# drscotthawley/signaltrain

Hardware: AMD Instinct MI355X
Metric: audio-frames/sec (train step) comp_4c 8192-sample windows @ 1/2/4/8 GPUs (higher is better)
Workload: dtype f32; 1 GPU; comp_4c synthetic, 8192-sample windows, batch 256/GPU, fp32 (BASELINE configs[1]); window=8192, frames_per_window=25, global_batch=256, parallelism=dp1

## Files before the change

### signaltrain_amd/csrc/st_ae.h

```cpp
#pragma once
#include "st_common.h"

namespace sta {

constexpr int NL = 9;
#ifndef ST_AE_ABLATE
#define ST_AE_ABLATE 0
#endif

struct AEOffsets { int w[NL]; int b[NL]; };

struct GroupWalk { int first, end, stride; };
__device__ __forceinline__ GroupWalk fwd_group_walk(const int ngroups, const int NW, const int wave)
{
    const int G = (int)gridDim.x, b = (int)blockIdx.x;
    if ((G & 7) == 0) {
        const int S = G >> 3, x = b & 7, slot = b >> 3;
        const int per = (ngroups + 7) >> 3;
        const int lo = x * per, hi = lo + per < ngroups ? lo + per : ngroups;
        return GroupWalk{lo + wave * S + slot, hi, S * NW};
    }
    return GroupWalk{wave * G + b, ngroups, G * NW};
}

struct CL {
    static constexpr int O0 = 64, O1 = 32, O2 = 16, O3 = 16, O4 = 16, O5 = 16, O6 = 32, O7 = 64, O8 = 16;
    static constexpr int I0 = 32, I1 = 64, I2 = 32, I3 = 16, I4 = 32, I5 = 16, I6 = 16, I7 = 32, I8 = 64;
    static constexpr int A0 = 0, A1 = A0 + O0 * I0, A2 = A1 + O1 * I1, A3 = A2 + O2 * I2, A4 = A3 + O3 * I3, A5 = A4 + O4 * I4,
                         A6 = A5 + O5 * I5, A7 = A6 + O6 * I6, A8 = A7 + O7 * I7, AEND = A8 + O8 * I8;
    static constexpr int B0 = AEND, B1 = B0 + O0, B2 = B1 + O1, B3 = B2 + O2, B4 = B3 + O3, B5 = B4 + O4, B6 = B5 + O5,
                         B7 = B6 + O6, B8 = B7 + O7, FWD_TOTAL = B8 + O8;
    static constexpr int G0 = FWD_TOTAL, G1 = G0 + O0 * I0, G2 = G1 + O1 * I1, G3 = G2 + O2 * I2, G4 = G3 + O3 * I3, G5 = G4 + O4 * I4,
                         G6 = G5 + O5 * I5, G7 = G6 + O6 * I6, G8 = G7 + O7 * I7, BWD_TOTAL = G8 + O8 * I8;
    static_assert(FWD_TOTAL % 4 == 0 && BWD_TOTAL % 4 == 0, "16-byte aligned regions");
};

constexpr int ae_max_elems(int l) { return l == 0 ? 64 * 32 : l == 1 ? 32 * 64 : l == 2 ? 16 * 32 : l == 3 ? 16 * 16 : l == 4 ? 16 * 32 :
                                           l == 5 ? 16 * 16 : l == 6 ? 32 * 16 : l == 7 ? 64 * 32 : 16 * 64; }
template <int NT>
struct AEParamRegs { float v[NL][(64 * 32 + NT - 1) / NT]; float bv[NL]; };

template <int NT>
__host__ __device__ __forceinline__ void ae_params_issue(AEParamRegs<NT>& r, const float* __restrict__ ae, const AEOffsets& go,
                                                const int T, const int OT, const int K, const int tid, const int l0, const int l1)
{
    const int out[NL] = {64, 32, 16, 16, 16, 16, 32, 64, OT};
    const int in[NL] = {T, 64, 32, 16, 16 + K, 16, 16, 32, 64};
#pragma unroll
    for (int l = 0; l < NL; ++l) {
        const bool on = l >= l0 && l < l1;
        const int n = on ? out[l] * in[l] : 0;
        const float* src = ae + go.w[l];
#pragma unroll
        for (int u = 0; u < (ae_max_elems(l) + NT - 1) / NT; ++u) { const int e = tid + u * NT; r.v[l][u] = src[e < n ? e : 0]; }
        r.bv[l] = ae[go.b[l] + (tid < out[l] ? tid : 0)];
    }
}
template <int BF> __device__ __forceinline__ unsigned short st_half_bits(const float v)
{
    if constexpr (BF == 2) { union { _Float16 h; unsigned short u; } p; p.h = (_Float16)v; return p.u; }
    else { union { __bf16 h; unsigned short u; } p; p.h = (__bf16)v; return p.u; }
}
template <int BF> __device__ __forceinline__ float st_half_to_float(const unsigned short b)
{
    if constexpr (BF == 2) { union { unsigned short u; _Float16 h; } p; p.u = b; return (float)p.h; }
    else return __uint_as_float((unsigned)b << 16);
}
template <int NT, int BF = 0>
__host__ __device__ __forceinline__ void ae_params_scatter(float* lds, const AEParamRegs<NT>& r, const int T, const int OT, const int K,
                                                  const int tid, const int l0, const int l1, const bool dgrad_images)
{
    const int out[NL] = {64, 32, 16, 16, 16, 16, 32, 64, OT};
    const int in[NL] = {T, 64, 32, 16, 16 + K, 16, 16, 32, 64};
    const int outp[NL] = {CL::O0, CL::O1, CL::O2, CL::O3, CL::O4, CL::O5, CL::O6, CL::O7, CL::O8};
    const int inp[NL] = {CL::I0, CL::I1, CL::I2, CL::I3, CL::I4, CL::I5, CL::I6, CL::I7, CL::I8};
    const int ao[NL] = {CL::A0, CL::A1, CL::A2, CL::A3, CL::A4, CL::A5, CL::A6, CL::A7, CL::A8};
    const int bo[NL] = {CL::B0, CL::B1, CL::B2, CL::B3, CL::B4, CL::B5, CL::B6, CL::B7, CL::B8};
    const int gi[NL] = {CL::G0, CL::G1, CL::G2, CL::G3, CL::G4, CL::G5, CL::G6, CL::G7, CL::G8};
#pragma unroll
    for (int l = 0; l < NL; ++l) {
        const bool on = l >= l0 && l < l1;
        const int IN = in[l], n = on ? out[l] * IN : 0, OP = outp[l], IP = inp[l];
#pragma unroll
        for (int u = 0; u < (ae_max_elems(l) + NT - 1) / NT; ++u) {
            const int e = tid + u * NT;
            if (e < n) {
                const int o = e / IN, i = e - o * IN;
                if constexpr (BF) {
                    const unsigned short hb = st_half_bits<BF>(r.v[l][u]);
                    reinterpret_cast<unsigned short*>(lds + ao[l])[(((i >> 2) * OP + o) << 2) + (i & 3)] = hb;
                    if (dgrad_images) reinterpret_cast<unsigned short*>(lds + gi[l])[(((o >> 2) * IP + i) << 2) + (o & 3)] = hb;
                } else {
                lds[ao[l] + (((i >> 2) * OP + o) << 2) + (i & 3)] = r.v[l][u];
                if (dgrad_images) lds[gi[l] + (((o >> 2) * IP + i) << 2) + (o & 3)] = r.v[l][u];
                }
            }
        }
        if (on && tid < out[l]) lds[bo[l] + tid] = r.bv[l];
    }
}
template <int NT, int BF = 0>
__device__ inline void ae_load_lds(float* lds, const float* __restrict__ ae, const AEOffsets& go, const int T, const int OT, const int K,
                                   const int tid, const int l0, const int l1, const bool dgrad_images)
{
    const int total = dgrad_images ? CL::BWD_TOTAL : CL::FWD_TOTAL;
#if ST_AE_ABLATE & 128
    for (int e = tid; e < total; e += NT) lds[e] = 0.f;
#else
    AEParamRegs<NT> r;
    ae_params_issue<NT>(r, ae, go, T, OT, K, tid, l0, l1);
    for (int e = tid; e < total; e += NT) lds[e] = 0.f;
    __syncthreads();
    ae_params_scatter<NT, BF>(lds, r, T, OT, K, tid, l0, l1, dgrad_images);
#endif
}
template <int NT, int BF = 0>
__device__ inline void ae_load_lds2(float* lds, const float* __restrict__ ae_m, const float* __restrict__ ae_p, const AEOffsets& go,
                                    const int T, const int OT, const int K, const int tid, const int l0, const int l1)
{
#if ST_AE_ABLATE & 128
    for (int e = tid; e < 2 * CL::FWD_TOTAL; e += NT) lds[e] = 0.f;
#else
    AEParamRegs<NT> rm, rp;
    ae_params_issue<NT>(rm, ae_m, go, T, OT, K, tid, l0, l1);
    ae_params_issue<NT>(rp, ae_p, go, T, OT, K, tid, l0, l1);
    for (int e = tid; e < 2 * CL::FWD_TOTAL; e += NT) lds[e] = 0.f;
    __syncthreads();
    ae_params_scatter<NT, BF>(lds, rm, T, OT, K, tid, l0, l1, false);
    ae_params_scatter<NT, BF>(lds + CL::FWD_TOTAL, rp, T, OT, K, tid, l0, l1, false);
#endif
}

constexpr int AE_IMG_DG = CL::BWD_TOTAL - CL::FWD_TOTAL;
__host__ __device__ constexpr int ae_img_fwd_floats(const int FP) { return 2 * CL::FWD_TOTAL + FP; }
__host__ __device__ constexpr int ae_img_floats(const int FP) { return ae_img_fwd_floats(FP) + 2 * AE_IMG_DG; }
struct AEImgJob { const float* ae[2]; float* img; AEOffsets go; int T, OT, K, F, FP; float expfac; int n, n_blk; };
__host__ __device__ __forceinline__ float ae_freq_weight(const float expfac, const int f) { return expf(expfac * (float)f); }
__host__ __device__ __forceinline__ void ae_img_build(const AEImgJob& j, const int p)
{
    if (p >= j.n) return;
    const int out[NL] = {64, 32, 16, 16, 16, 16, 32, 64, j.OT};
    const int in[NL] = {j.T, 64, 32, 16, 16 + j.K, 16, 16, 32, 64};
    const int outp[NL] = {CL::O0, CL::O1, CL::O2, CL::O3, CL::O4, CL::O5, CL::O6, CL::O7, CL::O8};
    const int inp[NL] = {CL::I0, CL::I1, CL::I2, CL::I3, CL::I4, CL::I5, CL::I6, CL::I7, CL::I8};
    const int ao[NL + 1] = {CL::A0, CL::A1, CL::A2, CL::A3, CL::A4, CL::A5, CL::A6, CL::A7, CL::A8, CL::AEND};
    const int bo[NL + 1] = {CL::B0, CL::B1, CL::B2, CL::B3, CL::B4, CL::B5, CL::B6, CL::B7, CL::B8, CL::FWD_TOTAL};
    float v = 0.f;
    const int q0 = p - 2 * CL::FWD_TOTAL;
    if (q0 >= 0 && q0 < j.FP) v = q0 < j.F ? ae_freq_weight(j.expfac, q0) : 0.f;
    else {
        const bool dg = q0 >= 0;
        const int net = dg ? (q0 - j.FP >= AE_IMG_DG) : (p >= CL::FWD_TOTAL);
        const int q = dg ? q0 - j.FP - net * AE_IMG_DG : p - net * CL::FWD_TOTAL;
        const float* __restrict__ ae = j.ae[net];
        if (!dg && q >= CL::AEND) {
#pragma unroll
            for (int l = 0; l < NL; ++l)
                if (q >= bo[l] && q < bo[l + 1]) { const int o = q - bo[l]; if (o < out[l]) v = ae[j.go.b[l] + o]; }
        } else {
#pragma unroll
            for (int l = 0; l < NL; ++l)
                if (q >= ao[l] && q < ao[l + 1]) {
                    const int s = (q - ao[l]) >> 2, lo = (q - ao[l]) & 3;
                    const int o = dg ? ((s / inp[l]) << 2) + lo : s % outp[l];
                    const int i = dg ? s % inp[l] : ((s / outp[l]) << 2) + lo;
                    if (o < out[l] && i < in[l]) v = ae[j.go.w[l] + o * in[l] + i];
                }
        }
    }
    j.img[p] = v;
}

#define ST_MFMA16(a, b, c) __builtin_amdgcn_mfma_f32_16x16x4f32((a), (b), (c), 0, 0, 0)

__device__ __forceinline__ float ldg32(const float* __restrict__ base, const unsigned elem)
{
    return *reinterpret_cast<const float*>(reinterpret_cast<const char*>(base) + (size_t)(elem << 2));
}
__device__ __forceinline__ void stg32(float* __restrict__ base, const unsigned elem, const float v)
{
    *reinterpret_cast<float*>(reinterpret_cast<char*>(base) + (size_t)(elem << 2)) = v;
}
#define ST_MUL24(a, b) __umul24((unsigned)(a), (unsigned)(b))

typedef short s16x4 __attribute__((ext_vector_type(4)));
typedef __bf16 bf16x4_t __attribute__((ext_vector_type(4)));
typedef _Float16 f16x4_t __attribute__((ext_vector_type(4)));
template <int BF>
__device__ __forceinline__ f32x4 mfma16h(const s16x4 a, const s16x4 b, const f32x4 c)
{
    if constexpr (BF == 2) {
        union { s16x4 s; f16x4_t h; } pa, pb; pa.s = a; pb.s = b;
        return __builtin_amdgcn_mfma_f32_16x16x16f16(pa.h, pb.h, c, 0, 0, 0);
    } else return __builtin_amdgcn_mfma_f32_16x16x16bf16_1k(a, b, c, 0, 0, 0);
}
#define ST_MFMA16B(a, b, c) mfma16h<BF>((a), (b), (c))
template <int BF>
__device__ __forceinline__ s16x4 pack_h4(f32x4 v)
{
    if constexpr (BF == 2) {
        union { f16x4_t h; s16x4 s; } p; p.h = __builtin_convertvector(v, f16x4_t); return p.s;
    } else {
        typedef __bf16 bf16x2_t __attribute__((ext_vector_type(2)));
        typedef float f32x2_t __attribute__((ext_vector_type(2)));
        union { bf16x2_t h; unsigned u; } lo, hi;
        lo.h = __builtin_convertvector((f32x2_t){v[0], v[1]}, bf16x2_t);
        hi.h = __builtin_convertvector((f32x2_t){v[2], v[3]}, bf16x2_t);
        union { unsigned u[2]; s16x4 s; } r; r.u[0] = lo.u; r.u[1] = hi.u; return r.s;
    }
}
#define pack_bf16x4(v) pack_h4<BF>(v)
template <int BF>
__device__ __forceinline__ float round_h(const float v)
{
    if constexpr (BF == 2) return (float)(_Float16)v;
    else {
        union { __bf16 h; unsigned short u; } p; p.h = (__bf16)v;
        union { unsigned u; float f; } q; q.u = (unsigned)p.u << 16; return q.f;
    }
}
#define bf16_rne(v) round_h<BF>(v)

template <int BF>
__device__ __forceinline__ f32x4 frag_read(const float* img, const int idx)
{
    if constexpr (BF) {
        typedef float f32x2_t __attribute__((ext_vector_type(2)));
        const f32x2_t lo = *reinterpret_cast<const f32x2_t*>(reinterpret_cast<const unsigned short*>(img) + idx);
        return __builtin_shufflevector(lo, lo, 0, 1, -1, -1);
    } else return *reinterpret_cast<const f32x4*>(img + idx);
}
__device__ __forceinline__ s16x4 frag_bits(const f32x4 v)
{
    typedef float f32x2_t __attribute__((ext_vector_type(2)));
    union { f32x2_t f; s16x4 s; } p; p.f = __builtin_shufflevector(v, v, 0, 1); return p.s;
}
template <int OUTP, int BF = 0>
__device__ __forceinline__ f32x4 frag_fwd(const float* img, const int ot, const int it, const int g, const int c)
{
    return frag_read<BF>(img, ((4 * it + g) * OUTP + 16 * ot + c) << 2);
}
template <int INP, int BF = 0>
__device__ __forceinline__ f32x4 frag_dgrad(const float* img, const int ot, const int it, const int g, const int c)
{
    return frag_read<BF>(img, ((4 * ot + g) * INP + 16 * it + c) << 2);
}

template <int NC, int OTL, int ITL, int OUTP, int BF = 0>
__device__ __forceinline__ void layer_fwd(const float* const (&W)[NC], const float* const (&bias)[NC],
                                          const f32x4 (&hin)[NC][ITL], f32x4 (&hout)[NC][OTL], const int g, const int c)
{
    s16x4 ph[NC][ITL];
    if constexpr (BF) {
#pragma unroll
        for (int ch = 0; ch < NC; ++ch)
#pragma unroll
            for (int it = 0; it < ITL; ++it) ph[ch][it] = pack_bf16x4(hin[ch][it]);
    }
#pragma unroll
    for (int ot = 0; ot < OTL; ++ot) {
        f32x4 acc[NC];
#pragma unroll
        for (int ch = 0; ch < NC; ++ch) acc[ch] = *reinterpret_cast<const f32x4*>(bias[ch] + 16 * ot + 4 * g);
#pragma unroll
        for (int it = 0; it < ITL; ++it) {
            f32x4 w[NC];
#pragma unroll
            for (int ch = 0; ch < NC; ++ch) w[ch] = frag_fwd<OUTP, BF>(W[ch], ot, it, g, c);
            if constexpr (BF) {
#pragma unroll
                for (int ch = 0; ch < NC; ++ch) acc[ch] = ST_MFMA16B(frag_bits(w[ch]), ph[ch][it], acc[ch]);
            } else {
#pragma unroll
                for (int r = 0; r < 4; ++r)
#pragma unroll
                    for (int ch = 0; ch < NC; ++ch) acc[ch] = ST_MFMA16(w[ch][r], hin[ch][it][r], acc[ch]);
            }
        }
#pragma unroll
        for (int ch = 0; ch < NC; ++ch) hout[ch][ot] = elu4(acc[ch]);
    }
}

template <int NC, int BF = 0>
__device__ __forceinline__ void layer5_fwd(const float* const (&lw)[NC], const f32x4 (&h4)[NC][1], const float (&kn)[4], const int KQ,
                                           f32x4 (&h5)[NC][1], const int g, const int c)
{
    f32x4 acc[NC], w[NC];
#pragma unroll
    for (int ch = 0; ch < NC; ++ch) { acc[ch] = *reinterpret_cast<const f32x4*>(lw[ch] + CL::B4 + 4 * g); w[ch] = frag_fwd<CL::O4, BF>(lw[ch] + CL::A4, 0, 0, g, c); }
    if constexpr (BF) {
#pragma unroll
        for (int ch = 0; ch < NC; ++ch) acc[ch] = ST_MFMA16B(frag_bits(w[ch]), pack_bf16x4(h4[ch][0]), acc[ch]);
    } else {
#pragma unroll
        for (int r = 0; r < 4; ++r)
#pragma unroll
            for (int ch = 0; ch < NC; ++ch) acc[ch] = ST_MFMA16(w[ch][r], h4[ch][0][r], acc[ch]);
    }
#pragma unroll
    for (int q = 0; q < 4; ++q)
        if (q < KQ) {
#pragma unroll
            for (int ch = 0; ch < NC; ++ch) {
                float wk;
                if constexpr (BF) wk = st_half_to_float<BF>(reinterpret_cast<const unsigned short*>(lw[ch] + CL::A4)[(((4 + q) * CL::O4 + c) << 2) + g]);
                else wk = lw[ch][CL::A4 + (((4 + q) * CL::O4 + c) << 2) + g];
                acc[ch] = ST_MFMA16(wk, BF ? bf16_rne(kn[q]) : kn[q], acc[ch]);
            }
        }
#pragma unroll
    for (int ch = 0; ch < NC; ++ch) h5[ch][0] = elu4(acc[ch]);
}

#define ST_W2(off_) {lw[0] + (off_), lw[1] + (off_)}

struct FwdIn { f32x4 v[2][2]; float tl[2][4]; float kn[4]; };

__device__ __forceinline__ void fwd_load_v(FwdIn& in, const float* __restrict__ mag, const float* __restrict__ phs,
                                           const int b, const int f, const bool fv, const int T, const int F, const int g)
{
    const unsigned base = ST_MUL24(ST_MUL24(b, T), F) + (unsigned)(fv ? f : 0);
#pragma unroll
// ... 275 lines not shown
#pragma unroll
        for (int it = 0; it < ITL; ++it) ph[it] = pack_bf16x4(hin[it]);
    }
#pragma unroll
    for (int ot = 0; ot < OTL; ++ot) {
        f32x4 acc = *reinterpret_cast<const f32x4*>(bias + 16 * ot + 4 * g);
#pragma unroll
        for (int it = 0; it < ITL; ++it) {
#if ST_AE_ABLATE & 32
            acc[0] += fr[ot * ITL + it][0] * hin[it][0];
#else
            if constexpr (BF) acc = ST_MFMA16B(frag_bits(fr[ot * ITL + it]), ph[it], acc);
            else {
#pragma unroll
                for (int r = 0; r < 4; ++r) acc = ST_MFMA16(fr[ot * ITL + it][r], hin[it][r], acc);
            }
#endif
        }
#if ST_AE_ABLATE & 8
#pragma unroll
        for (int r = 0; r < 4; ++r) hout[ot][r] = fmaxf(acc[r], 0.1f * acc[r]);
#else
        hout[ot] = elu4(acc);
#endif
    }
}
template <int TL>
__device__ __forceinline__ void to_T(float* scr, const f32x4 (&d)[TL], f32x4 (&t)[TL], const int g, const int c)
{
#if ST_AE_ABLATE & 16
#pragma unroll
    for (int k = 0; k < TL; ++k) t[k] = d[k];
    return;
#endif
#pragma unroll
    for (int k = 0; k < TL; ++k) *reinterpret_cast<f32x4*>(scr + k * 320 + c * 20 + 4 * g) = d[k];
#pragma unroll
    for (int k = 0; k < TL; ++k)
#pragma unroll
        for (int r = 0; r < 4; ++r) t[k][r] = scr[k * 320 + (4 * g + r) * 20 + c];
}

template <int BF> struct TTy { typedef f32x4 type; };
template <> struct TTy<1> { typedef s16x4 type; };
template <> struct TTy<2> { typedef s16x4 type; };
template <int TL, int BF>
__device__ __forceinline__ void to_Th(float* scr, const f32x4 (&d)[TL], typename TTy<BF>::type (&t)[TL], const int g, const int c)
{
    if constexpr (BF == 0) to_T<TL>(scr, d, t, g, c);
    else {
        short* hs = reinterpret_cast<short*>(scr);
#pragma unroll
        for (int k = 0; k < TL; ++k) *reinterpret_cast<s16x4*>(hs + k * 256 + c * 16 + 4 * g) = pack_h4<BF>(d[k]);
#pragma unroll
        for (int k = 0; k < TL; ++k)
            t[k] = __builtin_amdgcn_ds_read_tr16_b64_v4i16((s16x4 __attribute__((address_space(3)))*)(hs + k * 256 + (4 * g + (c >> 2)) * 16 + 4 * (c & 3)));
    }
}
template <int BF>
__device__ __forceinline__ typename TTy<BF>::type tt_splat(const float v)
{
    if constexpr (BF == 0) return (f32x4){v, v, v, v};
    else return pack_h4<BF>((f32x4){v, v, v, v});
}
template <int OTL, int ITL, int BF>
__device__ __forceinline__ void wgrad_regh(f32x4 (&dW)[OTL][ITL], float (&db)[OTL], const f32x4 (&daT)[OTL], const typename TTy<BF>::type (&hT)[ITL]);

template <int OTL, int ITL, int BF = 0>
__device__ __forceinline__ void dgradD_fr(const f32x4 (&fr)[ITL * OTL], const f32x4 (&da)[OTL], f32x4 (&dh)[ITL])
{
    s16x4 pd[OTL];
    if constexpr (BF) {
#pragma unroll
        for (int ot = 0; ot < OTL; ++ot) pd[ot] = pack_bf16x4(da[ot]);
    }
#pragma unroll
    for (int it = 0; it < ITL; ++it) {
        f32x4 acc = (f32x4){0.f, 0.f, 0.f, 0.f};
#pragma unroll
        for (int ot = 0; ot < OTL; ++ot) {
            if constexpr (BF) acc = ST_MFMA16B(frag_bits(fr[it * OTL + ot]), pd[ot], acc);
            else {
#pragma unroll
                for (int r = 0; r < 4; ++r) acc = ST_MFMA16(fr[it * OTL + ot][r], da[ot][r], acc);
            }
        }
        dh[it] = acc;
    }
}

template <int TL>
__device__ __forceinline__ void mul_elu_grad(f32x4 (&d)[TL], const f32x4 (&h)[TL])
{
#pragma unroll
    for (int t = 0; t < TL; ++t)
#pragma unroll
        for (int r = 0; r < 4; ++r) d[t][r] = __builtin_fmaf(d[t][r], __builtin_amdgcn_fmed3f(h[t][r], 0.f, -3.0e38f), d[t][r]);
}

template <int OTL, int ITL, int BF = 0>
__device__ __forceinline__ void wgrad_reg(f32x4 (&dW)[OTL][ITL], float (&db)[OTL], const f32x4 (&daT)[OTL], const f32x4 (&hT)[ITL])
{
    s16x4 pht[ITL];
    if constexpr (BF) {
#pragma unroll
        for (int it = 0; it < ITL; ++it) pht[it] = pack_bf16x4(hT[it]);
    }
#pragma unroll
    for (int ot = 0; ot < OTL; ++ot) {
        s16x4 pdt;
        if constexpr (BF) pdt = pack_bf16x4(daT[ot]);
#pragma unroll
        for (int it = 0; it < ITL; ++it) {
#if ST_AE_ABLATE & 4
            dW[ot][it][0] += daT[ot][0] * hT[it][0];
#else
            if constexpr (BF) dW[ot][it] = ST_MFMA16B(pdt, pht[it], dW[ot][it]);
            else {
#pragma unroll
                for (int r = 0; r < 4; ++r) dW[ot][it] = ST_MFMA16(daT[ot][r], hT[it][r], dW[ot][it]);
            }
#endif
        }
        db[ot] += (daT[ot][0] + daT[ot][1]) + (daT[ot][2] + daT[ot][3]);
    }
}
template <int OTL, int ITL, int BF>
__device__ __forceinline__ void wgrad_regh(f32x4 (&dW)[OTL][ITL], float (&db)[OTL], const f32x4 (&daT)[OTL], const typename TTy<BF>::type (&hT)[ITL])
{
    if constexpr (BF == 0) wgrad_reg<OTL, ITL, 0>(dW, db, daT, hT);
    else {
#pragma unroll
        for (int ot = 0; ot < OTL; ++ot) {
            const s16x4 pdt = pack_bf16x4(daT[ot]);
#pragma unroll
            for (int it = 0; it < ITL; ++it) dW[ot][it] = ST_MFMA16B(pdt, hT[it], dW[ot][it]);
            db[ot] += (daT[ot][0] + daT[ot][1]) + (daT[ot][2] + daT[ot][3]);
        }
    }
}
template <int OTL, int ITL, int INP, bool FIRST>
__device__ __forceinline__ void dw_flush(float* dW, const f32x4 (&acc)[OTL][ITL], const int g, const int c)
{
#pragma unroll
    for (int ot = 0; ot < OTL; ++ot)
#pragma unroll
        for (int it = 0; it < ITL; ++it)
#pragma unroll
            for (int r = 0; r < 4; ++r) {
                float* p = dW + (16 * ot + 4 * g + r) * INP + 16 * it + c;
                if constexpr (FIRST) *p = acc[ot][it][r]; else *p += acc[ot][it][r];
            }
}
template <int OTL, bool FIRST>
__device__ __forceinline__ void db_flush(float* dst, float (&db)[OTL], const int g, const int c)
{
#pragma unroll
    for (int ot = 0; ot < OTL; ++ot) {
        float v = db[ot];
        v += __shfl_xor(v, 16); v += __shfl_xor(v, 32);
        if (g == 0) { if constexpr (FIRST) dst[16 * ot + c] = v; else dst[16 * ot + c] += v; }
    }
}

__device__ __forceinline__ void group_colsum_store(float* __restrict__ dst, const f32x4& t, const int g, const int c)
{
    const float v = (t[0] + t[1]) + (t[2] + t[3]);
    const unsigned u = __builtin_bit_cast(unsigned, v);
    const auto p = __builtin_amdgcn_permlane16_swap(u, u, false, false);
    const float w = __builtin_bit_cast(float, (unsigned)p[0]) + __builtin_bit_cast(float, (unsigned)p[1]);
    const unsigned x = __builtin_bit_cast(unsigned, w);
    const auto q = __builtin_amdgcn_permlane32_swap(x, x, false, false);
    const float s = __builtin_bit_cast(float, (unsigned)q[0]) + __builtin_bit_cast(float, (unsigned)q[1]);
    if (g == 0) dst[c] = s;
}

constexpr int AE_BWD_SCR = (32 + 16 + 16) * SP + 2 * 4 * 320;
constexpr int ae_bwd_lds_floats(int nw) { return (CL::BWD_TOTAL + nw * AE_BWD_SCR) > nw * CL::FWD_TOTAL ? (CL::BWD_TOTAL + nw * AE_BWD_SCR) : nw * CL::FWD_TOTAL; }
template <int NW, bool INNER = false, int BF = 0, int VAR = 1, bool SAVED = false, bool KG = false, bool IMG = false>
__global__ void __launch_bounds__(NW * 64, 1)
ae_bwd_kernel(const float* __restrict__ mag, const float* __restrict__ phs, const float* __restrict__ knobs,
              const float* __restrict__ ae_m, const float* __restrict__ ae_p, const AEOffsets go, const int PG,
              const float* __restrict__ mag_hat, const float* __restrict__ phs_hat, const float* __restrict__ dAA,
              const float* __restrict__ g_mag_hat, const float reg_coef, const float expfac,
              float* __restrict__ dmag, float* __restrict__ dphs, float* __restrict__ ws,
              const int B, const int T, const int OT, const int F, const int K, const int KP,
              const int to_lo, const int to_hi,
              const int nslab, const size_t slab,
              const float* __restrict__ sv = nullptr,
              float* __restrict__ kg = nullptr,
              const float* __restrict__ img = nullptr)
{
    static_assert(!SAVED || (!INNER && BF == 0), "the kept-activation backward exists for the fused fp32 geometries");
    static_assert(!IMG || SAVED, "ready-made images: the kept-activation backward only");
    extern __shared__ __attribute__((aligned(16))) float lds[];
    const int ae = blockIdx.y;
    const int tid = threadIdx.x, lane = tid & 63, wave = tid >> 6;
    const int g = lane >> 4, c = lane & 15;
    float* lw = lds;
    float* Vs = lds + CL::BWD_TOTAL + wave * AE_BWD_SCR;
    float* Ys = Vs + 32 * SP;
    float* Ts = Ys + 16 * SP;
    float* XH = Ts + 16 * SP;
    float* XD = XH + 4 * 320;
    if constexpr (IMG && !(ST_AE_ABLATE & 128)) {
        const int FPi = KP / 2;
        const float* const dg = img + 2 * CL::FWD_TOTAL + FPi + ae * AE_IMG_DG;
        constexpr int N4 = AE_IMG_DG / 4, U = (N4 + NW * 64 - 1) / (NW * 64);
        f32x4 v[U];
#pragma unroll
        for (int u = 0; u < U; ++u) { const int e = tid + u * NW * 64; v[u] = reinterpret_cast<const f32x4*>(dg)[e < N4 ? e : 0]; }
        for (int i = tid; i < FPi / 4; i += NW * 64) reinterpret_cast<f32x4*>(lds)[i] = reinterpret_cast<const f32x4*>(img + 2 * CL::FWD_TOTAL)[i];
#pragma unroll
        for (int u = 0; u < U; ++u) { const int e = tid + u * NW * 64; if (e < N4) reinterpret_cast<f32x4*>(lds + CL::G0)[e] = v[u]; }
    } else
    ae_load_lds<NW * 64, BF>(lw, ae ? ae_p : ae_m, go, INNER ? 16 : T, INNER ? 16 : OT, K, tid, INNER ? 1 : 0, INNER ? 8 : NL, true);
    __syncthreads();

    const float* vin = ae ? phs : mag;
    const float* dh8in = ae ? phs_hat : mag_hat;
    float* dvout = ae ? dphs : dmag;
    const int FP = KP / 2, gpw = FP / 16;
    const int ngroups = B * gpw;
    const int gstride = gridDim.x * NW;

    f32x4 rW1[4][2], rW2[2][4], rW3[1][2], rW4[1][1], rW5[1][2], rW6[1][1], rW7[2][1], rW8[4][2], rW9[1][4];
    float rb1[4], rb2[2], rb3[1], rb4[1], rb5[1], rb6[1], rb7[2], rb8[4], rb9[1];
#define ST_ZT(x, A, Bq) { _Pragma("unroll") for (int a_ = 0; a_ < A; ++a_) _Pragma("unroll") for (int b_ = 0; b_ < Bq; ++b_) x[a_][b_] = (f32x4){0.f, 0.f, 0.f, 0.f}; }
#define ST_ZB(x, A) { _Pragma("unroll") for (int a_ = 0; a_ < A; ++a_) x[a_] = 0.f; }
    ST_ZT(rW1, 4, 2) ST_ZT(rW2, 2, 4) ST_ZT(rW3, 1, 2) ST_ZT(rW4, 1, 1) ST_ZT(rW5, 1, 2) ST_ZT(rW6, 1, 1) ST_ZT(rW7, 2, 1) ST_ZT(rW8, 4, 2) ST_ZT(rW9, 1, 4)
    ST_ZB(rb1, 4) ST_ZB(rb2, 2) ST_ZB(rb3, 1) ST_ZB(rb4, 1) ST_ZB(rb5, 1) ST_ZB(rb6, 1) ST_ZB(rb7, 2) ST_ZB(rb8, 4) ST_ZB(rb9, 1)
#undef ST_ZT
#undef ST_ZB

    f32x4 vr[2];
    int grp = blockIdx.x * NW + wave;
    auto load_v = [&](int gq, f32x4 (&dst)[2]) {
        const int bq = gq / gpw, fq = (gq - bq * gpw) * 16 + c;
        const unsigned base = ST_MUL24(ST_MUL24(bq, T), F) + (unsigned)(fq < F ? fq : 0);
#pragma unroll
        for (int it = 0; it < 2; ++it)
#pragma unroll
            for (int r = 0; r < 4; ++r) {
                const int t = 16 * it + 4 * g + r;
                dst[it][r] = ldg32(vin, base + ST_MUL24(t < T ? t : 0, F));
            }
    };
    auto mask_v = [&](int gq, f32x4 (&dst)[2]) {
        const int bq = gq / gpw, fq = (gq - bq * gpw) * 16 + c;
        const bool ok0 = fq < F;
#pragma unroll
        for (int it = 0; it < 2; ++it)
#pragma unroll
            for (int r = 0; r < 4; ++r) dst[it][r] = (ok0 && 16 * it + 4 * g + r < T) ? dst[it][r] : 0.f;
    };
    if constexpr (!INNER) { if (grp < ngroups) { load_v(grp, vr); mask_v(grp, vr); } }
    f32x4 kn = (f32x4){0.f, 0.f, 0.f, 0.f}; float knT = 0.f;
    auto load_kn = [&](int gq, f32x4& d4, float& dT) {
        const unsigned kb = ST_MUL24(gq / gpw, K);
#pragma unroll
        for (int r = 0; r < 4; ++r) { const int kidx = 4 * g + r; d4[r] = ldg32(knobs, kb + (unsigned)(kidx < K ? kidx : 0)); }
        dT = ldg32(knobs, kb + (unsigned)(c < K ? c : 0));
    };
    auto mask_kn = [&](f32x4& d4, float& dT) {
#pragma unroll
        for (int r = 0; r < 4; ++r) d4[r] = (4 * g + r) < K ? d4[r] : 0.f;
        dT = c < K ? dT : 0.f;
    };
    if (grp < ngroups) { load_kn(grp, kn, knT); mask_kn(kn, knT); }
    const unsigned Rw = (unsigned)B * FP;

    constexpr bool GM = (VAR & 1) != 0, TAIL16 = (VAR & 2) != 0;
    float q_x[4][3], q_y[4][3], q_ph[4], q_mh[4], q_mt[4], q_gm[4];
    auto load_q = [&](const int gq) {
        const int bq = gq / gpw, fq0 = (gq - bq * gpw) * 16 + c;
        const bool fvq = fq0 < F;
        const int fq = fvq ? fq0 : 0;
        const size_t o1 = nslab > 1 ? slab : 0, o2 = nslab > 2 ? 2 * slab : 0;
        const float* const dA0 = dAA, * const dA1 = dAA + o1, * const dA2 = dAA + o2;
        const float* const dB0 = dA0 + FP, * const dB1 = dA1 + FP, * const dB2 = dA2 + FP;
        const unsigned bOT = ST_MUL24(bq, OT), btF = ST_MUL24(ST_MUL24(bq, T), F) + (unsigned)fq;
#pragma unroll
        for (int r = 0; r < 4; ++r) {
            const int to = 4 * g + r;
            const bool ok = fvq && to < OT;
            const bool lv = ok && to >= to_lo && to <= to_hi;
            const unsigned ro = bOT + (unsigned)(ok ? to : 0);
            const unsigned p0 = ST_MUL24(lv ? ro : 0u, KP) + (unsigned)fq;
            const unsigned pF = ST_MUL24(ro, F) + (unsigned)fq;
#if ST_AE_ABLATE & 1
            q_x[r][0] = q_x[r][1] = q_x[r][2] = q_y[r][0] = q_y[r][1] = q_y[r][2] = 1e-3f * (float)(p0 & 7); q_ph[r] = 0.3f; q_mh[r] = 0.2f + 1e-3f * (float)(pF & 3);
#else
            q_x[r][0] = ldg32(dA0, p0); q_x[r][1] = ldg32(dA1, p0); q_x[r][2] = ldg32(dA2, p0);
            q_y[r][0] = ldg32(dB0, p0); q_y[r][1] = ldg32(dB1, p0); q_y[r][2] = ldg32(dB2, p0);
            q_ph[r] = ldg32(phs_hat, pF); q_mh[r] = ldg32(mag_hat, pF);
#endif
            if constexpr (GM) q_gm[r] = ldg32(g_mag_hat, pF); else q_gm[r] = 0.f;
            if constexpr (!TAIL16) q_mt[r] = ldg32(vin, btF + ST_MUL24(ok ? T - OT + to : 0, F));
        }
    };
    f32x4 s_h1[4], s_h2[2], s_h3[1], s_h4[1], s_h5[1], s_h6[1], s_h7[2], s_h8[4], s_e9[1];
    const float* const svn = SAVED ? sv + (size_t)ae * ngroups * (AE_SV_TILES * 256) : nullptr;
    const unsigned lane16 = (unsigned)lane << 4;
#ifdef ST_SV_DIAG
    auto svp = [&](const int gq) { return svn + (size_t)(__builtin_amdgcn_readfirstlane(gq) & ST_SV_DIAG) * (AE_SV_TILES * 256); };
#else
    auto svp = [&](const int gq) { return svn + (size_t)__builtin_amdgcn_readfirstlane(gq) * (AE_SV_TILES * 256); };
#endif
    if constexpr (SAVED) {
        if (grp < ngroups) {
            load_q(grp);
            const float* const p = svp(grp);
            sv_load(p, lane16, 16, s_e9); sv_load(p, lane16, 12, s_h8); sv_load(p, lane16, 10, s_h7); sv_load(p, lane16, 9, s_h6); sv_load(p, lane16, 8, s_h5);
            sv_load(p, lane16, 7, s_h4); sv_load(p, lane16, 6, s_h3); sv_load(p, lane16, 4, s_h2); sv_load(p, lane16, 0, s_h1);
        }
    }

    for (; grp < ngroups; grp += gstride) {
        asm volatile("" ::: "memory");
        const int b = grp / gpw, f = (grp - b * gpw) * 16 + c;
        const bool fv = f < F;
        if constexpr (!INNER && !SAVED) load_q(grp);
        f32x4 h1in[4], dh8[4];
        if constexpr (INNER) {
            const unsigned col0 = (unsigned)b * FP + (unsigned)(grp - b * gpw) * 16;
#pragma unroll
            for (int ot = 0; ot < 4; ++ot) {
#pragma unroll
                for (int r = 0; r < 4; ++r) {
                    h1in[ot][r] = ldg32(vin, (unsigned)(16 * ot + 4 * g + r) * Rw + col0 + c);
                    dh8[ot][r] = ldg32(dh8in, (unsigned)(16 * ot + 4 * g + r) * Rw + col0 + c);
                }
            }
        }
        f32x4 vn[2], knn; float knTn;
        const int gnext = grp + gstride < ngroups ? grp + gstride : grp;
#if ST_AE_ABLATE & 64
        vn[0] = vr[0]; vn[1] = vr[1]; knn = kn; knTn = knT;
#else
        if constexpr (!INNER) load_v(gnext, vn);
        load_kn(gnext, knn, knTn);
#endif

        f32x4 h1[4], h2[2], h3[1], h4[1], h5[1], h6[1], h7[2], h8[4], e9[1];
        f32x4 fr9[1 * 4];
        if constexpr (SAVED) {
#pragma unroll
            for (int it = 0; it < 2; ++it)
#pragma unroll
                for (int r = 0; r < 4; ++r) Vs[(16 * it + 4 * g + r) * SP + c] = vr[it][r];
#pragma unroll
            for (int k = 0; k < 4; ++k) { h1[k] = s_h1[k]; h8[k] = s_h8[k]; }
#pragma unroll
            for (int k = 0; k < 2; ++k) { h2[k] = s_h2[k]; h7[k] = s_h7[k]; }
            h3[0] = s_h3[0]; h4[0] = s_h4[0]; h5[0] = s_h5[0]; h6[0] = s_h6[0]; e9[0] = s_e9[0];
        } else {
        f32x4 fr2[2 * 4];
        if constexpr (INNER) {
#pragma unroll
            for (int ot = 0; ot < 4; ++ot) h1[ot] = h1in[ot];
            frags_fwd<2, 4, CL::O1, BF>(fr2, lw + CL::A1, g, c);
        } else {
            f32x4 fr1[4 * 2]; frags_fwd<4, 2, CL::O0, BF>(fr1, lw + CL::A0, g, c);
            frags_fwd<2, 4, CL::O1, BF>(fr2, lw + CL::A1, g, c);
#pragma unroll
            for (int it = 0; it < 2; ++it)
#pragma unroll
                for (int r = 0; r < 4; ++r) Vs[(16 * it + 4 * g + r) * SP + c] = vr[it][r];
            ST_FENCE();
            fwdD_fr<4, 2, BF>(fr1, lw + CL::B0, vr, h1, g);
        }
        f32x4 fr3[1 * 2]; frags_fwd<1, 2, CL::O2, BF>(fr3, lw + CL::A2, g, c); ST_FENCE(); fwdD_fr<2, 4, BF>(fr2, lw + CL::B1, h1, h2, g);
        f32x4 fr4[1 * 1]; frags_fwd<1, 1, CL::O3, BF>(fr4, lw + CL::A3, g, c); ST_FENCE(); fwdD_fr<1, 2, BF>(fr3, lw + CL::B2, h2, h3, g);
        f32x4 fr5[1 * 2]; frags_fwd<1, 2, CL::O4, BF>(fr5, lw + CL::A4, g, c); ST_FENCE(); fwdD_fr<1, 1, BF>(fr4, lw + CL::B3, h3, h4, g);
        f32x4 fr6[1 * 1]; frags_fwd<1, 1, CL::O5, BF>(fr6, lw + CL::A5, g, c); ST_FENCE();
        {
            const f32x4 hk[2] = {h4[0], kn};
            fwdD_fr<1, 2, BF>(fr5, lw + CL::B4, hk, h5, g);
        }
        f32x4 fr7[2 * 1]; frags_fwd<2, 1, CL::O6, BF>(fr7, lw + CL::A6, g, c); ST_FENCE(); fwdD_fr<1, 1, BF>(fr6, lw + CL::B5, h5, h6, g);
        f32x4 fr8[4 * 2]; frags_fwd<4, 2, CL::O7, BF>(fr8, lw + CL::A7, g, c); ST_FENCE(); fwdD_fr<2, 1, BF>(fr7, lw + CL::B6, h6, h7, g);
        if constexpr (!INNER) frags_fwd<1, 4, CL::O8, BF>(fr9, lw + CL::A8, g, c);
        ST_FENCE(); fwdD_fr<4, 2, BF>(fr8, lw + CL::B7, h7, h8, g);
        }
        f32x4 da9[1];
        float dxA[4], mtA[4];
        if constexpr (!INNER) {
            ST_FENCE();
            float wf;
            if constexpr (IMG && !(ST_AE_ABLATE & 128)) wf = fv ? lds[f] : 0.f;
            else wf = fv ? ae_freq_weight(expfac, f) : 0.f;
#pragma unroll
            for (int r = 0; r < 4; ++r) {
                const int to = 4 * g + r;
                const bool ok = fv && to < OT;
                const bool lv = ok && to >= to_lo && to <= to_hi;
                const float gre = lv ? q_x[r][0] + (nslab > 1 ? q_x[r][1] : 0.f) + (nslab > 2 ? q_x[r][2] : 0.f) : 0.f;
                const float gim = lv ? q_y[r][0] + (nslab > 1 ? q_y[r][1] : 0.f) + (nslab > 2 ? q_y[r][2] : 0.f) : 0.f;
                const float ph = q_ph[r], mh = q_mh[r];
                if constexpr (!TAIL16) asm volatile("" :: "v"(q_mt[r]));
                float sn, cs; st_sincos(ph, sn, cs);
                const float sg = mh > 0.f ? 1.f : (mh < 0.f ? -1.f : 0.f);
                const float dmh = gre * cs + gim * sn + reg_coef * sg * wf + (GM ? q_gm[r] : 0.f);
                const float dph = mh * (gim * cs - gre * sn);
                dxA[r] = ok ? (ae == 0 ? dmh : dph) : 0.f;
                mtA[r] = ae == 0 ? (TAIL16 ? vr[1][r] : q_mt[r]) : 1.f;
            }
            if constexpr (!SAVED) fwdD_fr<1, 4, BF>(fr9, lw + CL::B8, h8, e9, g);
            if constexpr (BF == 0 && !SAVED) {
#pragma unroll
                for (int p_ = 0; p_ < 16; ++p_) { __builtin_amdgcn_sched_group_barrier(0x008, 1, 0); __builtin_amdgcn_sched_group_barrier(0x002, 7, 0); }
            }
            ST_FENCE();
        }
        if constexpr (!INNER) {
#pragma unroll
            for (int r = 0; r < 4; ++r) {
                const int to = 4 * g + r;
                const float eg = elu_grad_from_out(e9[0][r]);
                const float e1 = ae == 0 ? e9[0][r] : 1.f;
                const float d9 = dxA[r] * mtA[r] * eg;
                const float tail = dxA[r] * e1;
                da9[0][r] = d9;
                Ts[to * SP + c] = tail;
                Ys[to * SP + c] = d9;
            }
        }
#define ST_REFILL(...) do { if constexpr (SAVED) { ST_FENCE(); __VA_ARGS__; ST_FENCE(); } } while (0)
        const float* const svq = SAVED ? svp(gnext) : nullptr;
        ST_REFILL(load_q(gnext); sv_load(svq, lane16, 16, s_e9));
#define ST_PIPE(N_) do { \
        __builtin_amdgcn_sched_group_barrier(0x008, (N_) + 2, 0); \
        _Pragma("unroll") for (int p_ = 0; p_ < (N_) - 2; ++p_) { \
            __builtin_amdgcn_sched_group_barrier(0x002, 2, 0); __builtin_amdgcn_sched_group_barrier(0x300, 1, 0); \
            __builtin_amdgcn_sched_group_barrier(0x008, 1, 0); } \
        ST_FENCE(); } while (0)
#define ST_BWD_STAGE(O_, I_, FD_, DA_, DAT_, HP_, HTP_, DAP_, DATP_, RW_, RB_, NEXT_) \
        to_Th<I_, BF>(XH, HP_, HTP_, g, c); ST_FENCE(); \
        dgradD_fr<O_, I_, BF>(FD_, DA_, DAP_); mul_elu_grad<I_>(DAP_, HP_); \
        to_T<I_>(XD, DAP_, DATP_, g, c); NEXT_; \
        wgrad_regh<O_, I_, BF>(RW_, RB_, DAT_, HTP_); \
        ST_PIPE(BF ? O_ * I_ : O_ * I_ * 4);
        typedef typename TTy<BF>::type tt_t;
        tt_t hT8[4]; f32x4 da8[4], daT8[4], fd8[2 * 4];
        if constexpr (INNER) {
            frags_dgrad<4, 2, CL::I7, BF>(fd8, lw + CL::G7, g, c);
            to_Th<4, BF>(XH, h8, hT8, g, c);
#pragma unroll
            for (int ot = 0; ot < 4; ++ot) da8[ot] = dh8[ot];
            mul_elu_grad<4>(da8, h8); to_T<4>(XD, da8, daT8, g, c);
        } else {
            f32x4 daT9[1], fd9[4 * 1];
            frags_dgrad<1, 4, CL::I8, BF>(fd9, lw + CL::G8, g, c);
            daT9[0] = *reinterpret_cast<const f32x4*>(Ys + c * SP + 4 * g);
            ST_BWD_STAGE(1, 4, fd9, da9, daT9, h8, hT8, da8, daT8, rW9, rb9, (frags_dgrad<4, 2, CL::I7, BF>(fd8, lw + CL::G7, g, c)))
            ST_REFILL(sv_load(svq, lane16, 12, s_h8));
        }
        tt_t hT7[2]; f32x4 da7[2], daT7[2], fd7[1 * 2];
        ST_BWD_STAGE(4, 2, fd8, da8, daT8, h7, hT7, da7, daT7, rW8, rb8, (frags_dgrad<2, 1, CL::I6, BF>(fd7, lw + CL::G6, g, c)))
        ST_REFILL(sv_load(svq, lane16, 10, s_h7));
        tt_t hT6[1]; f32x4 da6[1], daT6[1], fd6[1];
        ST_BWD_STAGE(2, 1, fd7, da7, daT7, h6, hT6, da6, daT6, rW7, rb7, (frags_dgrad<1, 1, CL::I5, BF>(fd6, lw + CL::G5, g, c)))
        ST_REFILL(sv_load(svq, lane16, 9, s_h6));
        tt_t hT5[1]; f32x4 da5[1], daT5[1], fd5[1];
        ST_BWD_STAGE(1, 1, fd6, da6, daT6, h5, hT5, da5, daT5, rW6, rb6, (frags_dgrad<1, 1, CL::I4, BF>(fd5, lw + CL::G4, g, c)))
        ST_REFILL(sv_load(svq, lane16, 8, s_h5));
        tt_t hT4[1], hT4k[2]; f32x4 da4[1], daT4[1], fd4[1];
        {
            to_Th<1, BF>(XH, h4, hT4, g, c); ST_FENCE();
            dgradD_fr<1, 1, BF>(fd5, da5, da4); mul_elu_grad<1>(da4, h4);
            to_T<1>(XD, da4, daT4, g, c); frags_dgrad<1, 1, CL::I3, BF>(fd4, lw + CL::G3, g, c); ST_FENCE();
            hT4k[0] = hT4[0];
            hT4k[1] = tt_splat<BF>(knT);
            wgrad_regh<1, 2, BF>(rW5, rb5, daT5, hT4k);
            if constexpr (KG) group_colsum_store(kg + ((size_t)ae * ngroups + grp) * 16, daT5[0], g, c);
        }
        ST_REFILL(sv_load(svq, lane16, 7, s_h4));
        tt_t hT3[1]; f32x4 da3[1], daT3[1], fd3[2 * 1];
        ST_BWD_STAGE(1, 1, fd4, da4, daT4, h3, hT3, da3, daT3, rW4, rb4, (frags_dgrad<1, 2, CL::I2, BF>(fd3, lw + CL::G2, g, c)))
        ST_REFILL(sv_load(svq, lane16, 6, s_h3));
        tt_t hT2[2]; f32x4 da2[2], daT2[2], fd2[4 * 2];
        ST_BWD_STAGE(1, 2, fd3, da3, daT3, h2, hT2, da2, daT2, rW3, rb3, (frags_dgrad<2, 4, CL::I1, BF>(fd2, lw + CL::G1, g, c)))
        ST_REFILL(sv_load(svq, lane16, 4, s_h2));
        tt_t hT1[4]; f32x4 da1[4], daT1[4], fd1[2 * 4];
        if constexpr (INNER) {
            to_Th<4, BF>(XH, h1, hT1, g, c); ST_FENCE();
            dgradD_fr<2, 4, BF>(fd2, da2, da1); mul_elu_grad<4>(da1, h1);
            const unsigned col0 = (unsigned)b * FP + (unsigned)(grp - b * gpw) * 16;
#pragma unroll
            for (int ot = 0; ot < 4; ++ot)
#pragma unroll
                for (int r = 0; r < 4; ++r) stg32(dvout, (unsigned)(16 * ot + 4 * g + r) * Rw + col0 + c, da1[ot][r]);
            ST_FENCE();
            wgrad_regh<2, 4, BF>(rW2, rb2, daT2, hT1);
        } else {
            ST_BWD_STAGE(2, 4, fd2, da2, daT2, h1, hT1, da1, daT1, rW2, rb2, (frags_dgrad<4, 2, CL::I0, BF>(fd1, lw + CL::G0, g, c)))
            ST_REFILL(sv_load(svq, lane16, 0, s_h1));
        }
        f32x4 vT[2], dv[2];
        if constexpr (!INNER) {
#pragma unroll
            for (int it = 0; it < 2; ++it) vT[it] = *reinterpret_cast<const f32x4*>(Vs + (16 * it + c) * SP + 4 * g);
            ST_FENCE();
            dgradD_fr<4, 2, BF>(fd1, da1, dv);
            wgrad_reg<4, 2, BF>(rW1, rb1, daT1, vT);
        }
#undef ST_BWD_STAGE
#undef ST_PIPE
#undef ST_REFILL
        if constexpr (!INNER) {
            mask_v(gnext, vn);
            vr[0] = vn[0]; vr[1] = vn[1];
        }
        mask_kn(knn, knTn); kn = knn; knT = knTn;
        if constexpr (!INNER) {
        float dvs[2][4], tls[2][4];
#pragma unroll
        for (int it = 0; it < 2; ++it)
#pragma unroll
            for (int r = 0; r < 4; ++r) {
                dvs[it][r] = dv[it][r]; asm volatile("" : "+v"(dvs[it][r]));
                const int ti = 16 * it + 4 * g + r - (T - OT);
                tls[it][r] = Ts[(ti >= 0 && ti < OT ? ti : 0) * SP + c];
            }
        const unsigned dv0 = ST_MUL24(ST_MUL24(b, T), F) + (unsigned)f;
#pragma unroll
        for (int it = 0; it < 2; ++it)
#pragma unroll
            for (int r = 0; r < 4; ++r) {
                const int t = 16 * it + 4 * g + r;
                const float v = dvs[it][r] + (t >= T - OT ? tls[it][r] : 0.f);
#if ST_AE_ABLATE & 2
                asm volatile("" :: "v"(v));
#else
                if (fv && t < T) stg32(dvout, dv0 + ST_MUL24(t, F), v);
#endif
            }
        }
    }
#if ST_AE_ABLATE & 256
    {
#define ST_KT(x, A, Bq) { _Pragma("unroll") for (int a_ = 0; a_ < A; ++a_) _Pragma("unroll") for (int b_ = 0; b_ < Bq; ++b_) _Pragma("unroll") for (int r_ = 0; r_ < 4; ++r_) asm volatile("" :: "v"(x[a_][b_][r_])); }
#define ST_KB(x, A) { _Pragma("unroll") for (int a_ = 0; a_ < A; ++a_) asm volatile("" :: "v"(x[a_])); }
        ST_KT(rW1, 4, 2) ST_KT(rW2, 2, 4) ST_KT(rW3, 1, 2) ST_KT(rW4, 1, 1) ST_KT(rW5, 1, 2) ST_KT(rW6, 1, 1) ST_KT(rW7, 2, 1) ST_KT(rW8, 4, 2) ST_KT(rW9, 1, 4)
        ST_KB(rb1, 4) ST_KB(rb2, 2) ST_KB(rb3, 1) ST_KB(rb4, 1) ST_KB(rb5, 1) ST_KB(rb6, 1) ST_KB(rb7, 2) ST_KB(rb8, 4) ST_KB(rb9, 1)
#undef ST_KT
#undef ST_KB
        return;
    }
#endif
    __syncthreads();
    static_assert(NW == 4, "the store pass sums exactly four per-wave images");
    float* dwl = lds + wave * CL::FWD_TOTAL;
    if constexpr (!INNER) { dw_flush<4, 2, CL::I0, true>(dwl + CL::A0, rW1, g, c); dw_flush<1, 4, CL::I8, true>(dwl + CL::A8, rW9, g, c);
                            db_flush<4, true>(dwl + CL::B0, rb1, g, c); db_flush<1, true>(dwl + CL::B8, rb9, g, c); }
    dw_flush<2, 4, CL::I1, true>(dwl + CL::A1, rW2, g, c); dw_flush<1, 2, CL::I2, true>(dwl + CL::A2, rW3, g, c);
    dw_flush<1, 1, CL::I3, true>(dwl + CL::A3, rW4, g, c); dw_flush<1, 2, CL::I4, true>(dwl + CL::A4, rW5, g, c);
    dw_flush<1, 1, CL::I5, true>(dwl + CL::A5, rW6, g, c); dw_flush<2, 1, CL::I6, true>(dwl + CL::A6, rW7, g, c);
    dw_flush<4, 2, CL::I7, true>(dwl + CL::A7, rW8, g, c);
    db_flush<2, true>(dwl + CL::B1, rb2, g, c); db_flush<1, true>(dwl + CL::B2, rb3, g, c); db_flush<1, true>(dwl + CL::B3, rb4, g, c);
    db_flush<1, true>(dwl + CL::B4, rb5, g, c); db_flush<1, true>(dwl + CL::B5, rb6, g, c); db_flush<2, true>(dwl + CL::B6, rb7, g, c);
    db_flush<4, true>(dwl + CL::B7, rb8, g, c);
    __syncthreads();
    auto sum4 = [&](int idx) { return (lds[idx] + lds[CL::FWD_TOTAL + idx]) + (lds[2 * CL::FWD_TOTAL + idx] + lds[3 * CL::FWD_TOTAL + idx]); };
    float* base = ws + ((size_t)blockIdx.x * 2 + ae) * PG;
    const int out[NL] = {64, 32, 16, 16, 16, 16, 32, 64, OT};
    const int in[NL] = {T, 64, 32, 16, 16 + K, 16, 16, 32, 64};
    const int inp[NL] = {CL::I0, CL::I1, CL::I2, CL::I3, CL::I4, CL::I5, CL::I6, CL::I7, CL::I8};
    const int ao[NL] = {CL::A0, CL::A1, CL::A2, CL::A3, CL::A4, CL::A5, CL::A6, CL::A7, CL::A8};
    const int bo[NL] = {CL::B0, CL::B1, CL::B2, CL::B3, CL::B4, CL::B5, CL::B6, CL::B7, CL::B8};
    constexpr int NT = NW * 64;
#pragma unroll
    for (int l = 0; l < NL; ++l) {
        const bool have = !INNER || (l >= 1 && l < 8);
        const int IN = in[l], n = out[l] * IN;
#pragma unroll
        for (int u = 0; u < (ae_max_elems(l) + NT - 1) / NT; ++u) {
            const int e = tid + u * NT;
            if (e < n) { const int o = e / IN, i = e - o * IN; base[go.w[l] + e] = have ? sum4(ao[l] + o * inp[l] + i) : 0.f; }
        }
        if (tid < out[l]) base[go.b[l] + tid] = have ? sum4(bo[l] + tid) : 0.f;
        { const int p0 = go.w[l] + n, np = go.b[l] - p0; if (tid < np) base[p0 + tid] = 0.f; }
        { const int p0 = go.b[l] + out[l], np = (l + 1 < NL ? go.w[l + 1] : PG) - p0; if (tid < np) base[p0 + tid] = 0.f; }
    }
}

}
```

Before: 11.14 million frames/s.

## Store per-wave weight gradients in quad layout and defer next-group q loads

In the IMG path, per-wave weight-gradient accumulators for layers 0-7 are written to LDS as contiguous float4 quads instead of scattered scalars. The final four-wave reduction then reads float4 vectors and scatters the four rows to global memory. Separately, the prefetch of the next group's q values is moved later in the backward pass, after the layer-2 stage, to shorten register live ranges or overlap the loads better. The cost is that the new LDS layout has to match the offsets and padding assumptions exactly, and delaying the load risks exposing its latency.

```diff
diff --git a/signaltrain_amd/csrc/st_ae.h b/signaltrain_amd/csrc/st_ae.h
--- a/signaltrain_amd/csrc/st_ae.h
+++ b/signaltrain_amd/csrc/st_ae.h
@@ -169,6 +169,16 @@
         }
     }
     j.img[p] = v;
+}
+
+__host__ __device__ __forceinline__ int ae_quad_pos(const int INP, const int o, const int i)
+{
+    return (((o >> 2) * INP + i) << 2) | (o & 3);
+}
+__host__ __device__ __forceinline__ int ae_quad_slot_dest(const int INP, const int IN, const int s)
+{
+    const int i = s & (INP - 1), o4 = s / INP;
+    return i < IN ? (o4 << 2) * IN + i : -1;
 }
 
 #define ST_MFMA16(a, b, c) __builtin_amdgcn_mfma_f32_16x16x4f32((a), (b), (c), 0, 0, 0)
@@ -750,6 +760,34 @@
                 if constexpr (FIRST) *p = acc[ot][it][r]; else *p += acc[ot][it][r];
             }
 }
+template <int OTL, int ITL, int INP>
+__device__ __forceinline__ void dw_flush_quad(float* dW, const f32x4 (&acc)[OTL][ITL], const int g, const int c)
+{
+#pragma unroll
+    for (int ot = 0; ot < OTL; ++ot)
+#pragma unroll
+        for (int it = 0; it < ITL; ++it) *reinterpret_cast<f32x4*>(dW + ae_quad_pos(INP, 16 * ot + 4 * g, 16 * it + c)) = acc[ot][it];
+}
+template <int OUTP, int INP, int NT>
+__device__ __forceinline__ void pgrad_store_quad(const float* img, float* __restrict__ dst, const int IN, const int tid)
+{
+    constexpr int N4 = OUTP * INP / 4, U = (N4 + NT - 1) / NT;
+    f32x4 v[U];
+#pragma unroll
+    for (int u = 0; u < U; ++u) {
+        const int s = tid + u * NT, sc = (N4 % NT) ? (s < N4 ? s : 0) : s;
+        const f32x4* p = reinterpret_cast<const f32x4*>(img) + sc;
+        v[u] = (p[0] + p[CL::FWD_TOTAL / 4]) + (p[2 * (CL::FWD_TOTAL / 4)] + p[3 * (CL::FWD_TOTAL / 4)]);
+    }
+#pragma unroll
+    for (int u = 0; u < U; ++u) {
+        const int s = tid + u * NT, e = ae_quad_slot_dest(INP, IN, s);
+        if (s < N4 && e >= 0) {
+#pragma unroll
+            for (int r = 0; r < 4; ++r) stg32(dst, (unsigned)(e + r * IN), v[u][r]);
+        }
+    }
+}
 template <int OTL, bool FIRST>
 __device__ __forceinline__ void db_flush(float* dst, float (&db)[OTL], const int g, const int c)
 {
@@ -988,6 +1026,17 @@
             float wf;
             if constexpr (IMG && !(ST_AE_ABLATE & 128)) wf = fv ? lds[f] : 0.f;
             else wf = fv ? ae_freq_weight(expfac, f) : 0.f;
+#if ST_AE_ABLATE & 512
+            float qk[4];
+#pragma unroll
+            for (int r = 0; r < 4; ++r) {
+                qk[r] = 0.3f; asm volatile("" : "+v"(qk[r]));
+                asm volatile("" :: "a"(q_x[r][0])); asm volatile("" :: "a"(q_x[r][1])); asm volatile("" :: "a"(q_x[r][2]));
+                asm volatile("" :: "a"(q_y[r][0])); asm volatile("" :: "a"(q_y[r][1])); asm volatile("" :: "a"(q_y[r][2]));
+                asm volatile("" :: "a"(q_ph[r])); asm volatile("" :: "a"(q_mh[r]));
+                q_x[r][0] = q_x[r][1] = q_x[r][2] = q_y[r][0] = q_y[r][1] = q_y[r][2] = q_ph[r] = q_mh[r] = qk[r];
+            }
+#endif
 #pragma unroll
             for (int r = 0; r < 4; ++r) {
                 const int to = 4 * g + r;
@@ -1026,7 +1075,8 @@
         }
 #define ST_REFILL(...) do { if constexpr (SAVED) { ST_FENCE(); __VA_ARGS__; ST_FENCE(); } } while (0)
         const float* const svq = SAVED ? svp(gnext) : nullptr;
-        ST_REFILL(load_q(gnext); sv_load(svq, lane16, 16, s_e9));
+        constexpr bool Q_LATE = IMG && !(ST_AE_ABLATE & 512);
+        ST_REFILL(if constexpr (!Q_LATE) load_q(gnext); sv_load(svq, lane16, 16, s_e9));
 #define ST_PIPE(N_) do { \
         __builtin_amdgcn_sched_group_barrier(0x008, (N_) + 2, 0); \
         _Pragma("unroll") for (int p_ = 0; p_ < (N_) - 2; ++p_) { \
@@ -1093,7 +1143,7 @@
             wgrad_regh<2, 4, BF>(rW2, rb2, daT2, hT1);
         } else {
             ST_BWD_STAGE(2, 4, fd2, da2, daT2, h1, hT1, da1, daT1, rW2, rb2, (frags_dgrad<4, 2, CL::I0, BF>(fd1, lw + CL::G0, g, c)))
-            ST_REFILL(sv_load(svq, lane16, 0, s_h1));
+            ST_REFILL(sv_load(svq, lane16, 0, s_h1); if constexpr (Q_LATE) load_q(gnext));
         }
         f32x4 vT[2], dv[2];
         if constexpr (!INNER) {
@@ -1150,12 +1200,21 @@
     __syncthreads();
     static_assert(NW == 4, "the store pass sums exactly four per-wave images");
     float* dwl = lds + wave * CL::FWD_TOTAL;
+    if constexpr (IMG) {
+        dw_flush_quad<4, 2, CL::I0>(dwl + CL::A0, rW1, g, c); dw_flush<1, 4, CL::I8, true>(dwl + CL::A8, rW9, g, c);
+        db_flush<4, true>(dwl + CL::B0, rb1, g, c); db_flush<1, true>(dwl + CL::B8, rb9, g, c);
+        dw_flush_quad<2, 4, CL::I1>(dwl + CL::A1, rW2, g, c); dw_flush_quad<1, 2, CL::I2>(dwl + CL::A2, rW3, g, c);
+        dw_flush_quad<1, 1, CL::I3>(dwl + CL::A3, rW4, g, c); dw_flush_quad<1, 2, CL::I4>(dwl + CL::A4, rW5, g, c);
+        dw_flush_quad<1, 1, CL::I5>(dwl + CL::A5, rW6, g, c); dw_flush_quad<2, 1, CL::I6>(dwl + CL::A6, rW7, g, c);
+        dw_flush_quad<4, 2, CL::I7>(dwl + CL::A7, rW8, g, c);
+    } else {
     if constexpr (!INNER) { dw_flush<4, 2, CL::I0, true>(dwl + CL::A0, rW1, g, c); dw_flush<1, 4, CL::I8, true>(dwl + CL::A8, rW9, g, c);
                             db_flush<4, true>(dwl + CL::B0, rb1, g, c); db_flush<1, true>(dwl + CL::B8, rb9, g, c); }
     dw_flush<2, 4, CL::I1, true>(dwl + CL::A1, rW2, g, c); dw_flush<1, 2, CL::I2, true>(dwl + CL::A2, rW3, g, c);
     dw_flush<1, 1, CL::I3, true>(dwl + CL::A3, rW4, g, c); dw_flush<1, 2, CL::I4, true>(dwl + CL::A4, rW5, g, c);
     dw_flush<1, 1, CL::I5, true>(dwl + CL::A5, rW6, g, c); dw_flush<2, 1, CL::I6, true>(dwl + CL::A6, rW7, g, c);
     dw_flush<4, 2, CL::I7, true>(dwl + CL::A7, rW8, g, c);
+    }
     db_flush<2, true>(dwl + CL::B1, rb2, g, c); db_flush<1, true>(dwl + CL::B2, rb3, g, c); db_flush<1, true>(dwl + CL::B3, rb4, g, c);
     db_flush<1, true>(dwl + CL::B4, rb5, g, c); db_flush<1, true>(dwl + CL::B5, rb6, g, c); db_flush<2, true>(dwl + CL::B6, rb7, g, c);
     db_flush<4, true>(dwl + CL::B7, rb8, g, c);
@@ -1168,10 +1227,17 @@
     const int ao[NL] = {CL::A0, CL::A1, CL::A2, CL::A3, CL::A4, CL::A5, CL::A6, CL::A7, CL::A8};
     const int bo[NL] = {CL::B0, CL::B1, CL::B2, CL::B3, CL::B4, CL::B5, CL::B6, CL::B7, CL::B8};
     constexpr int NT = NW * 64;
+    if constexpr (IMG) {
+        pgrad_store_quad<CL::O0, CL::I0, NT>(lds + CL::A0, base + go.w[0], in[0], tid); pgrad_store_quad<CL::O1, CL::I1, NT>(lds + CL::A1, base + go.w[1], in[1], tid);
+        pgrad_store_quad<CL::O2, CL::I2, NT>(lds + CL::A2, base + go.w[2], in[2], tid); pgrad_store_quad<CL::O3, CL::I3, NT>(lds + CL::A3, base + go.w[3], in[3], tid);
+        pgrad_store_quad<CL::O4, CL::I4, NT>(lds + CL::A4, base + go.w[4], in[4], tid); pgrad_store_quad<CL::O5, CL::I5, NT>(lds + CL::A5, base + go.w[5], in[5], tid);
+        pgrad_store_quad<CL::O6, CL::I6, NT>(lds + CL::A6, base + go.w[6], in[6], tid); pgrad_store_quad<CL::O7, CL::I7, NT>(lds + CL::A7, base + go.w[7], in[7], tid);
+    }
 #pragma unroll
     for (int l = 0; l < NL; ++l) {
         const bool have = !INNER || (l >= 1 && l < 8);
         const int IN = in[l], n = out[l] * IN;
+        if (!(IMG && l < NL - 1))
 #pragma unroll
         for (int u = 0; u < (ae_max_elems(l) + NT - 1) / NT; ++u) {
             const int e = tid + u * NT;
```

Result: no change. 11.18 million frames/s (median of 2 runs) (+0.3%).
